# TonyLianLong/LLM-groundedDiffusion

Hardware: AMD Instinct MI355X
Metric: images/sec (50-step SD1.5 512^2, LMD+ guidance) (higher is better)
Workload: dtype fp16

## Files before the change

### llm-groundeddiffusion_amd/csrc/attn.hip

```cpp
#include <atomic>
#include "common.h"
#include "../../include/lgd_hip.h"
#include "attn_w4.h"
#include <stdlib.h>
#include <string.h>

namespace {

int g_attn32_nw = -1;
int attn32_nw() {
  if (g_attn32_nw < 0) { const char* e = getenv("LGD_ATTN32_NW"); g_attn32_nw = e ? atoi(e) : 8; }
  return g_attn32_nw;
}
int g_attn32_var = 0;
int attn32_var() { return g_attn32_var; }
int g_attn32 = -1;
int attn32_mode() {
  if (g_attn32 < 0) { const char* e = getenv("LGD_ATTN32"); g_attn32 = e ? atoi(e) : 1; }
  return g_attn32;
}

std::atomic<int> g_attn_w4{-1};
int attn_w4_mode() {
  int v = g_attn_w4.load(std::memory_order_relaxed);
// ... 791 lines not shown
    __syncthreads();
    if (t + 2 < n_tiles) load_k((t + 2) * KV_T);
    if (more) load_v((t + 1) * KV_T);
    const float mx_nxt = pipelined_tile((t + 1) & 1, t & 1, s_cur, s_nxt);
    if (more) {
      const float mx = mx_nxt;
      if (__builtin_amdgcn_ballot_w64(mx > 8.f) != 0) {
        const float m_new = (float)(half_t)fmaxf(m_ref, mx + m_ref);
        const float shift = m_new - m_ref;
        const float alpha = __builtin_amdgcn_exp2f(-shift);
#pragma unroll
        for (int dt = 0; dt < NDT; ++dt)
#pragma unroll
          for (int r = 0; r < 16; ++r) oacc[dt][r] *= alpha;
#pragma unroll
        for (int kb = 0; kb < 2; ++kb)
#pragma unroll
          for (int r = 0; r < 16; ++r) s_nxt[kb][r] -= shift;
        m_ref = m_new;
        set_ref(m_new);
      }
#pragma unroll
      for (int kb = 0; kb < 2; ++kb) s_cur[kb] = s_nxt[kb];
    }
  }

  float l;
  {
    const int dl = d & 31, dt_l = d >> 5, h_l = (dl >> 2) & 1, r_l = (dl & 3) + 4 * (dl >> 3);
    float lv = 0.f;
#pragma unroll
    for (int dt = 0; dt < NDT; ++dt)
#pragma unroll
      for (int r = 0; r < 16; ++r)
        if (dt == dt_l && r == r_l) lv = oacc[dt][r];
    l = __shfl(lv, h_l * 32 + qi, 64);
  }
  const int qrow = q0 + qi;
  if (qrow < a.Sq) {
    const float inv = 1.f / l;
    half_t* orow = a.o + (long)b * a.o_bs + (long)qrow * a.ldo + (long)h * d;
#pragma unroll
    for (int dt = 0; dt < NDT; ++dt)
#pragma unroll
      for (int g4 = 0; g4 < 4; ++g4) {
        const int dv = dt * 32 + g4 * 8 + hh * 4;
        if (dv < d) {
          half4_t o;
#pragma unroll
          for (int r = 0; r < 4; ++r) o[r] = (half_t)(oacc[dt][g4 * 4 + r] * inv);
          *reinterpret_cast<half4_t*>(orow + dv) = o;
        }
      }
    if (a.lse && hh == 0) a.lse[((long)b * a.H + h) * a.Sq + qrow] = m_ref + log2f(l);
  }
}

template <int DP, bool SAVE_P>
void launch_attn_dp(const AttnArgs& a, hipStream_t st) {
  if constexpr (SAVE_P) {
    dim3 grid((a.Sq + 63) / 64, a.H, a.B);
    hipLaunchKernelGGL((attn_fwd_kernel<DP>), grid, dim3(256), 0, st, a);
  } else {
    if constexpr (DP == 64 || DP == 96) {
      const int a32 = attn32_mode();
      const int dk = ((a.d + 2 + 15) / 16) * 16;
      const long blocks256 = (long)((a.Sq + 255) / 256) * a.H * a.B;
      if (a32 && a.d % 8 == 0 && (a32 == 2 || (dk == 96 && blocks256 >= 128))) {
        const int var = attn32_var();
        auto go = [&](auto kern, int nw) {
          dim3 g32((a.Sq + 32 * nw - 1) / (32 * nw), a.H, a.B);
          hipLaunchKernelGGL(kern, g32, dim3(64 * nw), 0, st, a);
        };
        if (attn32_nw() == 4 || (a32 != 2 && blocks256 < 256)) {
          if (dk == 48) { go(&attn_self32_kernel<48, 2, 4>, 4); return; }
          if (dk == 96) { go(&attn_self32_kernel<96, 3, 4>, 4); return; }
        } else if (var == 1) {
          if (dk == 48) { go(&attn_self32_kernel<48, 2, 8, 4, true>, 8); return; }
          if (dk == 96) { go(&attn_self32_kernel<96, 3, 8, 4, true>, 8); return; }
        } else if (var == 2) {
          if (dk == 48) { go(&attn_self32_kernel<48, 2, 8, 2, false>, 8); return; }
          if (dk == 96) { go(&attn_self32_kernel<96, 3, 8, 2, false>, 8); return; }
        } else {
          if (dk == 48) { go(&attn_self32_kernel<48, 2, 8>, 8); return; }
          if (dk == 96) { go(&attn_self32_kernel<96, 3, 8>, 8); return; }
        }
      }
    }
    const bool qt2 = (long)((a.Sq + 127) / 128) * a.H * a.B >= 1024 && DP <= 96;
    dim3 grid(qt2 ? (a.Sq + 127) / 128 : (a.Sq + 63) / 64, a.H, a.B);
    if constexpr (DP <= 96) {
      static const int nw_env = [] { const char* e = getenv("LGD_ATTN_NW"); return e ? atoi(e) : 0; }();
      const bool nw8 = nw_env ? nw_env == 8 : ((DP == 64 && a.d < 48) || DP == 96);
      if (qt2 && nw8 && (long)((a.Sq + 255) / 256) * a.H * a.B >= 512) {
        dim3 g8((a.Sq + 255) / 256, a.H, a.B);
        if (DP == 64 && a.d < 48) hipLaunchKernelGGL((attn_self_kernel<DP, true, 2, DP == 64 ? 3 : DP / 16, 8>), g8, dim3(512), 0, st, a);
        else if (a.d < DP) hipLaunchKernelGGL((attn_self_kernel<DP, true, 2, DP / 16, 8>), g8, dim3(512), 0, st, a);
        else hipLaunchKernelGGL((attn_self_kernel<DP, false, 2, DP / 16, 8>), g8, dim3(512), 0, st, a);
        return;
      }
      if (qt2) {
        if (DP == 64 && a.d < 48) hipLaunchKernelGGL((attn_self_kernel<DP, true, 2, DP == 64 ? 3 : DP / 16>), grid, dim3(256), 0, st, a);
        else if (a.d < DP) hipLaunchKernelGGL((attn_self_kernel<DP, true, 2>), grid, dim3(256), 0, st, a);
        else hipLaunchKernelGGL((attn_self_kernel<DP, false, 2>), grid, dim3(256), 0, st, a);
        return;
      }
    }
    if constexpr (DP == 160) {
      static const int wide = [] { const char* e = getenv("LGD_ATTN160"); return e ? atoi(e) : 1; }();
      if (wide && a.d == DP && a.Sq >= 256 && (long)a.H * a.B * ((a.Sq + 63) / 64) > 256) {
        dim3 g8((a.Sq + 255) / 256, a.H, a.B);
        hipLaunchKernelGGL((attn_self_kernel<DP, false, 2, DP / 16, 8>), g8, dim3(512), 0, st, a);
        return;
      }
    }
    if (DP == 64 && a.d < 48) hipLaunchKernelGGL((attn_self_kernel<DP, true, 1, DP == 64 ? 3 : DP / 16>), grid, dim3(256), 0, st, a);
    else if (a.d < DP) hipLaunchKernelGGL((attn_self_kernel<DP, true, 1>), grid, dim3(256), 0, st, a);
    else hipLaunchKernelGGL((attn_self_kernel<DP, false, 1>), grid, dim3(256), 0, st, a);
  }
}

template <bool SAVE_P>
int launch_attn(const AttnArgs& a, hipStream_t st) {
  const int d = a.d;
  if constexpr (!SAVE_P) {
    const int w4 = attn_w4_mode();
    if (w4 && d == 40) {
      AttnW4Args w;
      w.q = a.q; w.ldq = a.ldq; w.q_bs = a.q_bs; w.k = a.k; w.ldk = a.ldk; w.k_bs = a.k_bs;
      w.v = a.v; w.ldv = a.ldv; w.v_bs = a.v_bs; w.o = a.o; w.ldo = a.ldo; w.o_bs = a.o_bs; w.lse = a.lse;
      w.B = a.B; w.H = a.H; w.Sq = a.Sq; w.Sk = a.Sk; w.d = a.d; w.scale_log2 = a.scale_log2;
      const long wgs = (long)((a.Sq + 255) / 256) * a.H * a.B;
      if (lgd_attn_w4_supported(w) && (w4 == 2 || (wgs >= 256 && a.Sk >= 256))) return lgd_attn_w4_launch(w, st);
    }
  }
  if (d <= 32) launch_attn_dp<32, SAVE_P>(a, st);
  else if (d <= 64) launch_attn_dp<64, SAVE_P>(a, st);
  else if (d <= 96) launch_attn_dp<96, SAVE_P>(a, st);
  else if (d <= 128) launch_attn_dp<128, SAVE_P>(a, st);
  else if (d <= 160) launch_attn_dp<160, SAVE_P>(a, st);
  else if (d <= 192) launch_attn_dp<192, SAVE_P>(a, st);
  else return LGD_ERR_UNSUPPORTED;
  return lgd_check_launch();
}

bool bad_view(int64_t ld, int d) { return (ld % 8) != 0 || (d % 8) != 0; }

}

void lgd_gn_set_fused_hw(int hw);
void lgd_gn_set_slab(int on);
void lgd_ln_set_stream(int on);
void lgd_gn_set_apply_wgs(int n);

extern "C" int lgd_set_option(const char* name, int value) {
  if (!name) return LGD_ERR_ARG;
  if (!strcmp(name, "gn_fused") && value >= 0 && value <= 4096) { lgd_gn_set_fused_hw(value); return LGD_OK; }
  if (!strcmp(name, "gn_slab") && (value == 0 || value == 1)) { lgd_gn_set_slab(value); return LGD_OK; }
  if (!strcmp(name, "ln_stream") && (value == 0 || value == 1)) { lgd_ln_set_stream(value); return LGD_OK; }
  if (!strcmp(name, "gn_apply_wgs") && value >= 64 && value <= 8192) { lgd_gn_set_apply_wgs(value); return LGD_OK; }
  if (!strcmp(name, "attn32")) { g_attn32 = value; return LGD_OK; }
  if (!strcmp(name, "attn_w4") && value >= 0 && value <= 2) { g_attn_w4.store(value, std::memory_order_relaxed); return LGD_OK; }
  if (!strcmp(name, "attn_w4_pipe") && (value == 0 || value == 1)) { lgd_attn_w4_set_pipe(value); return LGD_OK; }
  if (!strcmp(name, "attn32_nw") && (value == 4 || value == 8)) { g_attn32_nw = value; return LGD_OK; }
  if (!strcmp(name, "attn32_var") && value >= 0 && value <= 2) { g_attn32_var = value; return LGD_OK; }
  return LGD_ERR_ARG;
}

extern "C" int lgd_attn_fwd_f16(const void* q, int64_t ldq, int64_t q_bs, const void* k,
                                int64_t ldk, int64_t k_bs, const void* v, int64_t ldv, int64_t v_bs,
                                void* o, int64_t ldo, int64_t o_bs, float* lse, int B, int H, int Sq,
                                int Sk, int d, float scale, void* stream) {
  (void)hipGetLastError();
  if (B < 1 || H < 1 || Sq < 1 || Sk < 1 || d < 8) return LGD_ERR_ARG;
  if (bad_view(ldq, d) || bad_view(ldk, d) || bad_view(ldv, d) || (ldo % 4)) return LGD_ERR_ARG;
  AttnArgs a;
  a.q = (const half_t*)q; a.ldq = ldq; a.q_bs = q_bs;
  a.k = (const half_t*)k; a.ldk = ldk; a.k_bs = k_bs;
  a.v = (const half_t*)v; a.ldv = ldv; a.v_bs = v_bs;
  a.o = (half_t*)o; a.ldo = ldo; a.o_bs = o_bs;
  a.lse = lse; a.probs = nullptr; a.tok = -1; a.cond_only = 0; a.causal = 0;
  a.B = B; a.H = H; a.Sq = Sq; a.Sk = Sk; a.d = d;
  a.scale_log2 = scale * 1.4426950408889634f;
  return launch_attn<false>(a, reinterpret_cast<hipStream_t>(stream));
}

extern "C" int lgd_cross_attn_fwd_f16(const void* q, int64_t ldq, int64_t q_bs, const void* k,
                                      int64_t ldk, int64_t k_bs, const void* v, int64_t ldv,
                                      int64_t v_bs, void* o, int64_t ldo, int64_t o_bs, float* probs,
                                      int tok, int cond_only, int B, int H, int Sq, int Sk, int d,
                                      float scale, void* stream) {
  (void)hipGetLastError();
  if (B < 1 || H < 1 || Sq < 1 || Sk < 1 || d < 8) return LGD_ERR_ARG;
  if (bad_view(ldq, d) || bad_view(ldk, d) || bad_view(ldv, d) || (ldo % 4)) return LGD_ERR_ARG;
  if (cond_only && (B % 2)) return LGD_ERR_ARG;
  if (tok >= Sk) return LGD_ERR_ARG;
  AttnArgs a;
  a.q = (const half_t*)q; a.ldq = ldq; a.q_bs = q_bs;
  a.k = (const half_t*)k; a.ldk = ldk; a.k_bs = k_bs;
  a.v = (const half_t*)v; a.ldv = ldv; a.v_bs = v_bs;
  a.o = (half_t*)o; a.ldo = ldo; a.o_bs = o_bs;
  a.lse = nullptr; a.probs = probs; a.tok = tok; a.cond_only = cond_only; a.causal = 0;
  a.B = B; a.H = H; a.Sq = Sq; a.Sk = Sk; a.d = d;
  a.scale_log2 = scale * 1.4426950408889634f;
  hipStream_t st = reinterpret_cast<hipStream_t>(stream);
  if (probs) return launch_attn<true>(a, st);
  return launch_attn<false>(a, st);
}

extern "C" int lgd_attn_causal_fwd_f16(const void* q, int64_t ldq, int64_t q_bs, const void* k, int64_t ldk,
                                       int64_t k_bs, const void* v, int64_t ldv, int64_t v_bs, void* o,
                                       int64_t ldo, int64_t o_bs, int B, int H, int S, int d, float scale,
                                       void* stream) {
  (void)hipGetLastError();
  if (B < 1 || H < 1 || S < 1 || d < 8) return LGD_ERR_ARG;
  if (bad_view(ldq, d) || bad_view(ldk, d) || bad_view(ldv, d) || (ldo % 4)) return LGD_ERR_ARG;
  AttnArgs a;
  a.q = (const half_t*)q; a.ldq = ldq; a.q_bs = q_bs;
  a.k = (const half_t*)k; a.ldk = ldk; a.k_bs = k_bs;
  a.v = (const half_t*)v; a.ldv = ldv; a.v_bs = v_bs;
  a.o = (half_t*)o; a.ldo = ldo; a.o_bs = o_bs;
  a.lse = nullptr; a.probs = nullptr; a.tok = -1; a.cond_only = 0; a.causal = 1;
  a.B = B; a.H = H; a.Sq = S; a.Sk = S; a.d = d;
  a.scale_log2 = scale * 1.4426950408889634f;
  return launch_attn<true>(a, reinterpret_cast<hipStream_t>(stream));
}
```

### llm-groundeddiffusion_amd/csrc/gemm.hip

```cpp
#include "common.h"
#include "../../include/lgd_hip.h"
#include <map>
#include <mutex>
#include <utility>
#include <stdlib.h>

namespace {

constexpr int BK = 64;
constexpr int LDS_LD = BK + 16;

struct GemmArgs {
  LgdGemmDesc d;
  int cin;
  int k_per_split;
  int group_m;
#ifdef LGD_GEMM_ABLATION
  int stagger;
#endif
};

__device__ __forceinline__ float4 ld_bias4(const float* p, int n) {
  return *reinterpret_cast<const float4*>(p + n);
}

__device__ __forceinline__ f32x4 rownorm4(const LgdGemmDesc& d, int m, int n_in, f32x4 v) {
  if (d.epi & LGD_EPI_ROWNORM) {
    const float2 st = *reinterpret_cast<const float2*>(d.rowstat + (long)m * 2);
    const float4 cs = *reinterpret_cast<const float4*>(d.colsum + n_in);
    v[0] = st.y * (v[0] - st.x * cs.x); v[1] = st.y * (v[1] - st.x * cs.y);
    v[2] = st.y * (v[2] - st.x * cs.z); v[3] = st.y * (v[3] - st.x * cs.w);
  }
  return v;
}

template <bool GEGLU>
__device__ __forceinline__ f32x4 epilogue_value4(const LgdGemmDesc& d, long r_off, int m, int n_out, f32x4 v, f32x4 g,
                                                 float4 bv, float4 bg, bool res_ready, half4_t res_pre) {
  v[0] += bv.x; v[1] += bv.y; v[2] += bv.z; v[3] += bv.w;
  if (GEGLU) {
    g[0] += bg.x; g[1] += bg.y; g[2] += bg.z; g[3] += bg.w;
#ifdef LGD_GEMM_ABLATION
    if (d.epi & (1 << 16)) {
#pragma unroll
      for (int r = 0; r < 4; ++r) v[r] = v[r] * g[r];
    } else
#endif
    {
      const f32x2_t g01 = gelu2_f((f32x2_t){g[0], g[1]}), g23 = gelu2_f((f32x2_t){g[2], g[3]});
      v[0] *= g01[0]; v[1] *= g01[1]; v[2] *= g23[0]; v[3] *= g23[1];
    }
  }
  const float alpha = d.alpha;
#pragma unroll
  for (int r = 0; r < 4; ++r) v[r] *= alpha;
  if (res_ready) {
#pragma unroll
    for (int r = 0; r < 4; ++r) v[r] += (float)res_pre[r];
  } else if (d.res) {
    if (d.epi & LGD_EPI_RES_F32) {
      const float* rp = reinterpret_cast<const float*>(d.res) + r_off + (long)m * d.ldr + n_out;
      float4 rv = *reinterpret_cast<const float4*>(rp);
      v[0] += rv.x; v[1] += rv.y; v[2] += rv.z; v[3] += rv.w;
    } else {
      const half_t* rp = reinterpret_cast<const half_t*>(d.res) + r_off + (long)m * d.ldr + n_out;
      half4_t rv = *reinterpret_cast<const half4_t*>(rp);
#pragma unroll
      for (int r = 0; r < 4; ++r) v[r] += (float)rv[r];
    }
  }
  return v;
}

template <bool GEGLU>
__device__ __forceinline__ void epilogue_store4(const LgdGemmDesc& d, long c_off, long r_off, int m,
                                                int n_out, f32x4 v, f32x4 g, float4 bv, float4 bg,
                                                bool res_ready = false,
                                                half4_t res_pre = (half4_t){0, 0, 0, 0}) {
  v = epilogue_value4<GEGLU>(d, r_off, m, n_out, v, g, bv, bg, res_ready, res_pre);
  if (d.epi & LGD_EPI_OUT_F32) {
    float* cp = reinterpret_cast<float*>(d.c) + c_off + (long)m * d.ldc + n_out;
    *reinterpret_cast<float4*>(cp) = make_float4(v[0], v[1], v[2], v[3]);
  } else {
    half_t* cp = reinterpret_cast<half_t*>(d.c) + c_off + (long)m * d.ldc + n_out;
    half4_t o;
#pragma unroll
    for (int r = 0; r < 4; ++r) o[r] = (half_t)v[r];
    *reinterpret_cast<half4_t*>(cp) = o;
  }
}

__device__ __forceinline__ float4 ld_bias_sum4(const LgdGemmDesc& d, int n) {
  float4 b = make_float4(0.f, 0.f, 0.f, 0.f);
  if (d.bias) b = ld_bias4(d.bias, n);
  if (d.bias2) {
    float4 b2 = ld_bias4(d.bias2, n);
    b.x += b2.x; b.y += b2.y; b.z += b2.z; b.w += b2.w;
  }
  return b;
}

template <int MI, int NI>
__device__ __forceinline__ void gemm_epilogue(const GemmArgs& ga, f32x4 (&acc)[NI][MI], int m0, int n0,
                                              int wm, int wn, int lane, int batch, int split,
                                              long c_off, long r_off, int* lds_flag = nullptr) {
  const LgdGemmDesc& d = ga.d;
  const int m_l = lane & 15;
  const int n_l = (lane >> 4) * 4;
  if (d.splits > 1) {
    float* ws = ga.d.ws + ((long)batch * d.splits + split) * (long)d.M * d.N;
#pragma unroll
    for (int mi = 0; mi < MI; ++mi) {
      int m = m0 + wm * 16 * MI + mi * 16 + m_l;
      if (m >= d.M) continue;
#pragma unroll
      for (int ni = 0; ni < NI; ++ni) {
        int n = n0 + wn * 16 * NI + ni * 16 + n_l;
        if (n >= d.N) continue;
        f32x4 v = acc[ni][mi];
        *reinterpret_cast<float4*>(ws + (long)m * d.N + n) = make_float4(v[0], v[1], v[2], v[3]);
      }
    }
    if (!d.cnt || !lds_flag) return;
    asm volatile("s_waitcnt vmcnt(0)" ::: "memory");
    __syncthreads();
    int32_t* cnt = d.cnt + (long)batch * gridDim.x + blockIdx.x;
    if (threadIdx.x == 0) {
      __builtin_amdgcn_fence(__ATOMIC_RELEASE, "agent");
      asm volatile("s_waitcnt vmcnt(0)" ::: "memory");
      *lds_flag = __hip_atomic_fetch_add(cnt, 1, __ATOMIC_RELAXED, __HIP_MEMORY_SCOPE_AGENT);
    }
    __syncthreads();
    if (*lds_flag != d.splits - 1) return;
    if (threadIdx.x == 0) {
      __builtin_amdgcn_fence(__ATOMIC_ACQUIRE, "agent");
      __hip_atomic_store(cnt, 0, __ATOMIC_RELAXED, __HIP_MEMORY_SCOPE_AGENT);
    }
    __syncthreads();
    const float* w0 = ga.d.ws + (long)batch * d.splits * (long)d.M * d.N;
#pragma unroll
    for (int mi = 0; mi < MI; ++mi) {
      const int m = m0 + wm * 16 * MI + mi * 16 + m_l;
#pragma unroll
      for (int ni = 0; ni < NI; ++ni) {
        const int n = n0 + wn * 16 * NI + ni * 16 + n_l;
        f32x4 v = {0.f, 0.f, 0.f, 0.f};
        if (m < d.M && n < d.N) {
          for (int s2 = 0; s2 < d.splits; ++s2) {
            const float4 t = *reinterpret_cast<const float4*>(w0 + (long)s2 * d.M * d.N + (long)m * d.N + n);
            v[0] += t.x; v[1] += t.y; v[2] += t.z; v[3] += t.w;
          }
        }
        acc[ni][mi] = v;
      }
    }
  }
  const bool geglu = d.epi & LGD_EPI_GEGLU;
  if (geglu) {
// ... 1258 lines not shown
  const int frow = lane & 15, fg = lane >> 4, fsw = (frow >> 1) & 7;
  const unsigned lds0 = (unsigned)(uintptr_t)smem;
  unsigned a_ad0 = lds0 + (grp * 16 * MH + frow) * 128 + ((0 + fg) ^ fsw) * 16;
  unsigned a_ad1 = lds0 + (grp * 16 * MH + frow) * 128 + ((4 + fg) ^ fsw) * 16;
  unsigned b_ad0 = lds0 + OFF_B0 + (wn * 16 + frow) * 128 + ((0 + fg) ^ fsw) * 16;
  unsigned b_ad1 = lds0 + OFF_B0 + (wn * 16 + frow) * 128 + ((4 + fg) ^ fsw) * 16;
  using seqA = std::make_integer_sequence<int, MH>;
  using seqB0 = std::make_integer_sequence<int, NI0>;
  using seqB1 = std::make_integer_sequence<int, NI1>;

  f32x4 acc[NI][MI];
  half8_t af[2][MH], bf0[2][NI0], bf1[2][NI1];
  if constexpr (ABL & 2) {
#pragma unroll
    for (int kk = 0; kk < 2; ++kk) {
#pragma unroll
      for (int i = 0; i < MH; ++i) af[kk][i] = (half8_t){1, 1, 1, 1, 1, 1, 1, 1};
#pragma unroll
      for (int i = 0; i < NI0; ++i) bf0[kk][i] = (half8_t){1, 1, 1, 1, 1, 1, 1, 1};
#pragma unroll
      for (int i = 0; i < NI1; ++i) bf1[kk][i] = (half8_t){1, 1, 1, 1, 1, 1, 1, 1};
    }
  }

#define LGD_PH_MMA(BF, NB, NOFF, MOFF)                                                                              \
  {                                                                                                                 \
    asm volatile("s_waitcnt lgkmcnt(0)" ::: "memory");                                                              \
    __builtin_amdgcn_sched_barrier(0);                                                                              \
    if constexpr (!(ABL & 32)) __builtin_amdgcn_s_setprio(1);                                                       \
    _Pragma("unroll") for (int kk = 0; kk < 2; ++kk)                                                                \
      _Pragma("unroll") for (int ni = 0; ni < NB; ++ni)                                                             \
        _Pragma("unroll") for (int mi = 0; mi < MH; ++mi)                                                           \
          if constexpr (ABL & 4) asm volatile("" : "+v"(acc[NOFF + ni][MOFF + mi]) : "v"(BF[kk][ni]), "v"(af[kk][mi]));                \
          else acc[NOFF + ni][MOFF + mi] = __builtin_amdgcn_mfma_f32_16x16x32_f16(BF[kk][ni], af[kk][mi], acc[NOFF + ni][MOFF + mi], 0, 0, 0); \
    if constexpr (!(ABL & 32)) __builtin_amdgcn_s_setprio(0);                                                       \
    __builtin_amdgcn_sched_barrier(0);                                                                              \
  }
#define LGD_PH_BAR()                        \
  {                                         \
    __builtin_amdgcn_sched_barrier(0);      \
    __builtin_amdgcn_s_barrier();           \
    __builtin_amdgcn_sched_barrier(0);      \
  }

  if (nk > 0) {
    {
      unsigned sa, sw; int tap;
      k_pos(0, sa, sw, tap);
      dma_b(0, 0, true, sw, false);
      dma_a(0, 0, true, sa, tap, false);
      dma_b(1, 0, true, sw, false);
      dma_a(1, 0, true, sa, tap, false);
      k_pos(1, sa, sw, tap);
      dma_b(0, STAGE_B, nk > 1, sw, false);
      dma_a(0, STAGE_B, nk > 1, sa, tap, false);
    }
#pragma unroll
    for (int ni = 0; ni < NI; ++ni)
#pragma unroll
      for (int mi = 0; mi < MI; ++mi) acc[ni][mi] = (f32x4){0.f, 0.f, 0.f, 0.f};
    asm volatile("s_waitcnt vmcnt(%0)" ::"n"(T_DMA) : "memory");
    LGD_PH_BAR();
    if (grp == 1 && !(ABL & 64)) LGD_PH_BAR();
    unsigned so_cur = 0, so_nxt = STAGE_B;
    int sdelta = STAGE_B;
    for (int kt = 0; kt < nk; ++kt) {
      unsigned sa1, sw1, sa2, sw2; int tap1, tap2;
      k_pos(kt + 1, sa1, sw1, tap1);
      k_pos(kt + 2, sa2, sw2, tap2);
      const bool live1 = kt + 1 < nk, live2 = kt + 2 < nk;
      if constexpr (!(ABL & 2)) lds_read_frags<0, 64 * 128>(bf0[0], b_ad0, seqB0{});
      if constexpr (!(ABL & 2)) lds_read_frags<0, 64 * 128>(bf0[1], b_ad1, seqB0{});
      if constexpr (!(ABL & 2)) lds_read_frags<0, 16 * 128>(af[0], a_ad0, seqA{});
      if constexpr (!(ABL & 2)) lds_read_frags<0, 16 * 128>(af[1], a_ad1, seqA{});
      dma_b(1, so_nxt, live1, sw1);
      asm volatile("s_waitcnt vmcnt(%0)" ::"n"(T_DMA) : "memory");
      LGD_PH_BAR();
      LGD_PH_MMA(bf0, NI0, 0, 0);
      LGD_PH_BAR();
      if constexpr (!(ABL & 2)) lds_read_frags<BQ0_B, 64 * 128>(bf1[0], b_ad0, seqB1{});
      if constexpr (!(ABL & 2)) lds_read_frags<BQ0_B, 64 * 128>(bf1[1], b_ad1, seqB1{});
      dma_a(1, so_nxt, live1, sa1, tap1);
      asm volatile("s_waitcnt vmcnt(%0)" ::"n"(T_DMA) : "memory");
      LGD_PH_BAR();
      LGD_PH_MMA(bf1, NI1, NI0, 0);
      LGD_PH_BAR();
      if constexpr (!(ABL & 2)) lds_read_frags<OFF_A1, 16 * 128>(af[0], a_ad0, seqA{});
      if constexpr (!(ABL & 2)) lds_read_frags<OFF_A1, 16 * 128>(af[1], a_ad1, seqA{});
      dma_b(0, so_cur, live2, sw2);
      LGD_PH_BAR();
      LGD_PH_MMA(bf1, NI1, NI0, MH);
      LGD_PH_BAR();
      dma_a(0, so_cur, live2, sa2, tap2);
      asm volatile("s_waitcnt vmcnt(%0)" ::"n"(T_DMA) : "memory");
      LGD_PH_BAR();
      LGD_PH_MMA(bf0, NI0, 0, MH);
      LGD_PH_BAR();
      a_ad0 += sdelta; a_ad1 += sdelta; b_ad0 += sdelta; b_ad1 += sdelta;
      sdelta = -sdelta;
      const unsigned t = so_cur; so_cur = so_nxt; so_nxt = t;
    }
    if (grp == 0 && !(ABL & 64)) LGD_PH_BAR();
    asm volatile("s_waitcnt vmcnt(0) lgkmcnt(0)" ::: "memory");
    LGD_PH_BAR();
  }
  else {
#pragma unroll
    for (int ni = 0; ni < NI; ++ni)
#pragma unroll
      for (int mi = 0; mi < MI; ++mi) acc[ni][mi] = (f32x4){0.f, 0.f, 0.f, 0.f};
  }
#undef LGD_PH_MMA
#undef LGD_PH_BAR

  if constexpr (ABL & 16) {
#pragma unroll
    for (int ni = 0; ni < NI; ++ni)
#pragma unroll
      for (int mi = 0; mi < MI; ++mi) asm volatile("" ::"v"(acc[ni][mi]));
    return;
  }
  if (d.splits > 1) {
    const int m_l = lane & 15, n_l = (lane >> 4) * 4;
    float* ws = d.ws + ((long)batch * d.splits + split) * (long)d.M * d.N;
#pragma unroll
    for (int mi = 0; mi < MI; ++mi) {
      const int m = m0 + grp * 16 * MI + mi * 16 + m_l;
      if (m >= d.M) continue;
#pragma unroll
      for (int ni = 0; ni < NI; ++ni) {
        const int n = n0 + wn * 16 * NI + ni * 16 + n_l;
        if (n >= d.N) continue;
        const f32x4 v = acc[ni][mi];
        *reinterpret_cast<float4*>(ws + (long)m * d.N + n) = make_float4(v[0], v[1], v[2], v[3]);
      }
    }
    return;
  }
#define LGD_EPI_LDS(G, RS, RNORM) \
  gemm_epilogue_lds<MI, NI, WM, WN, (MI * NI > 32 ? STAGE_B : 2 * STAGE_B), G, true, RS, RNORM>(ga, acc, m0, n0, grp, wn, lane, tid, c_off, r_off, lds)
  const bool rn_ = d.epi & LGD_EPI_ROWNORM;
  if (d.epi & LGD_EPI_GEGLU) {
    if constexpr (NI % 2 == 0) {
      if (rn_) LGD_EPI_LDS(true, false, true); else LGD_EPI_LDS(true, false, false);
    }
  } else if (d.res) {
    if (rn_) LGD_EPI_LDS(false, true, true); else LGD_EPI_LDS(false, true, false);
  } else {
    if (rn_) LGD_EPI_LDS(false, false, true); else LGD_EPI_LDS(false, false, false);
  }
#undef LGD_EPI_LDS
}

__global__ __launch_bounds__(256) void splitk_reduce_kernel(const GemmArgs ga) {
  const LgdGemmDesc& d = ga.d;
  const bool geglu = d.epi & LGD_EPI_GEGLU;
  const int n_out_cols = geglu ? d.N / 2 : d.N;
  const long groups_per_row = n_out_cols / 4;
  const long total = (long)d.M * groups_per_row;
  const int batch = blockIdx.z;
  const int b_o = batch / d.nb_i, b_i = batch - b_o * d.nb_i;
  const long c_off = b_o * d.c_bs_o + b_i * d.c_bs_i;
  const long r_off = b_o * d.r_bs_o + b_i * d.r_bs_i;
  const float* ws = d.ws + (long)batch * d.splits * (long)d.M * d.N;
  for (long idx = blockIdx.x * 256L + threadIdx.x; idx < total; idx += (long)gridDim.x * 256L) {
    int m = (int)(idx / groups_per_row);
    int gcol = (int)(idx - (long)m * groups_per_row) * 4;
    int n_in = geglu ? (gcol / 16) * 32 + (gcol % 16) : gcol;
    f32x4 v = {0.f, 0.f, 0.f, 0.f}, g = {0.f, 0.f, 0.f, 0.f};
    for (int s = 0; s < d.splits; ++s) {
      const float* p = ws + (long)s * d.M * d.N + (long)m * d.N + n_in;
      float4 t = *reinterpret_cast<const float4*>(p);
      v[0] += t.x; v[1] += t.y; v[2] += t.z; v[3] += t.w;
      if (geglu) {
        float4 u = *reinterpret_cast<const float4*>(p + 16);
        g[0] += u.x; g[1] += u.y; g[2] += u.z; g[3] += u.w;
      }
    }
    const float4 bv = ld_bias_sum4(d, n_in);
    v = rownorm4(d, m, n_in, v);
    if (geglu) {
      float4 bg = make_float4(0.f, 0.f, 0.f, 0.f);
      if (d.bias) bg = ld_bias4(d.bias, n_in + 16);
      epilogue_store4<true>(d, c_off, r_off, m, gcol, v, rownorm4(d, m, n_in + 16, g), bv, bg);
    } else {
      epilogue_store4<false>(d, c_off, r_off, m, gcol, v, g, bv, bv);
    }
  }
}

enum GemmLoop : int {
  LOOP_REG,
  LOOP_DMA,
  LOOP_DMA8,
  LOOP_PIPE,
  LOOP_PHASE,
};
enum : unsigned {
  TILE_GEGLU = 1,
  TILE_PLAIN = 2,
  TILE_ONE_SPLIT = 4,
  TILE_LDS_EPI = 8,
  TILE_CONV_SAME = 16,
  TILE_CNT = 32,
};
struct GemmTile {
  int code;
  GemmLoop loop;
  int bm, bn;
  unsigned flags;
};
constexpr unsigned TILE_STD = TILE_GEGLU | TILE_CNT;
constexpr GemmTile GEMM_TILES[] = {
    {1, LOOP_REG, 128, 128, TILE_STD},   {2, LOOP_REG, 128, 64, TILE_STD},     {3, LOOP_REG, 64, 128, TILE_STD},
    {4, LOOP_REG, 64, 64, TILE_STD},     {5, LOOP_REG, 32, 128, TILE_STD},     {6, LOOP_REG, 128, 160, TILE_CNT},
    {7, LOOP_REG, 64, 160, TILE_CNT},
    {17, LOOP_DMA, 128, 128, TILE_STD},  {18, LOOP_DMA, 128, 64, TILE_STD},    {19, LOOP_DMA, 64, 128, TILE_STD},
    {20, LOOP_DMA, 64, 64, TILE_STD},    {21, LOOP_DMA, 32, 128, TILE_STD},    {22, LOOP_DMA, 128, 160, TILE_CNT},
    {23, LOOP_DMA, 64, 160, TILE_CNT},
    {25, LOOP_DMA8, 256, 320, TILE_CNT}, {26, LOOP_DMA8, 256, 128, TILE_STD},
    {33, LOOP_PIPE, 256, 160, TILE_CNT}, {34, LOOP_PIPE, 256, 128, TILE_STD}, {35, LOOP_PIPE, 256, 64, TILE_STD},
    {37, LOOP_PIPE, 128, 160, TILE_CNT}, {38, LOOP_PIPE, 128, 128, TILE_STD}, {39, LOOP_PIPE, 128, 64, TILE_STD},
    {40, LOOP_PIPE, 64, 160, TILE_CNT},  {41, LOOP_PIPE, 64, 128, TILE_STD},  {42, LOOP_PIPE, 64, 64, TILE_STD},
    {44, LOOP_PIPE, 256, 256, TILE_GEGLU | TILE_PLAIN | TILE_ONE_SPLIT | TILE_LDS_EPI},
    {45, LOOP_PIPE, 128, 128, TILE_STD | TILE_PLAIN},
    {46, LOOP_PHASE, 256, 256, TILE_GEGLU | TILE_LDS_EPI | TILE_CONV_SAME},
    {47, LOOP_PHASE, 256, 320, TILE_LDS_EPI | TILE_CONV_SAME},
};

const GemmTile* gemm_check(const LgdGemmDesc& desc, GemmArgs& ga) {
  ga.d = desc;
  LgdGemmDesc& d = ga.d;
  if (d.M <= 0 || d.N <= 0 || d.K <= 0) return nullptr;
  if (d.taps != 1 && d.taps != 9) return nullptr;
  ga.cin = d.c0 + d.c1;
  if (d.K != d.taps * ga.cin) return nullptr;
  if ((d.c0 % 8) || (d.c1 % 8) || (d.N % 4) || (d.ldw % 8) || (d.lda0 % 8) || (d.lda1 % 8) ||
      (d.ldc % 4))
    return nullptr;
  if (d.c1 > 0 && !d.a1) return nullptr;
  if (d.res && (d.ldr % 4)) return nullptr;
  if (d.nb_o < 1) d.nb_o = 1;
  if (d.nb_i < 1) d.nb_i = 1;
  if (d.splits < 1) d.splits = 1;
  const bool geglu = d.epi & LGD_EPI_GEGLU;
  if (geglu && (d.N % 32)) return nullptr;
  if (d.splits > 1 && !d.ws) return nullptr;
  if ((d.epi & LGD_EPI_ROWNORM) && (!d.rowstat || !d.colsum || d.taps != 1 || d.nb_o * d.nb_i != 1 || d.c1 > 0))
    return nullptr;
  int ktiles = (d.K + BK - 1) / BK;
  int tps = (ktiles + d.splits - 1) / d.splits;
  ga.k_per_split = tps * BK;
  d.splits = (ktiles + tps - 1) / tps;

  int code = d.tile;
  if (code == 0) {
    long batches = (long)d.nb_o * d.nb_i * d.splits;
    auto wgs = [&](int bm, int bn) {
      return batches * ((d.M + bm - 1) / bm) * ((d.N + bn - 1) / bn);
    };
    if (d.M <= 32) code = 21;
    else if (!geglu && d.N % 160 == 0 && wgs(128, 160) >= 384) code = 22;
    else if (!geglu && d.N % 160 == 0 && wgs(64, 160) >= 256) code = 23;
    else if (wgs(128, 128) >= 384 && d.N % 128 == 0) code = 17;
    else if (wgs(64, 128) >= 256 && d.N % 128 == 0) code = 19;
    else code = 20;
  }
  const GemmTile* t = nullptr;
  for (const GemmTile& e : GEMM_TILES)
    if (e.code == code) t = &e;
  if (!t) return nullptr;
  const unsigned f = t->flags;
  if (geglu && !(f & TILE_GEGLU)) return nullptr;
  if (t->loop == LOOP_DMA8 && (d.K % BK)) return nullptr;
  if ((t->loop == LOOP_PIPE || t->loop == LOOP_PHASE) && ((d.K % BK) || (ga.cin % BK) || (d.c0 % BK))) return nullptr;
  if ((f & TILE_PLAIN) && (d.taps != 1 || d.c1 > 0)) return nullptr;
  if (t->loop == LOOP_PHASE) {
    if (d.c1 > 0 || d.nb_o * d.nb_i != 1) return nullptr;
    if (((long)d.M + 2L * d.win + 2) * d.lda0 * 2 + 2L * d.K >= (1L << 31) || (long)d.N * d.ldw * 2 >= (1L << 31))
      return nullptr;
  }
  if ((f & TILE_CONV_SAME) && d.taps == 9 && (d.stride != 1 || d.ups != 0 || d.hin != d.hout || d.win != d.wout))
    return nullptr;
  if ((f & TILE_ONE_SPLIT) && d.splits != 1) return nullptr;
  if ((f & TILE_LDS_EPI) && d.splits == 1) {
    const long c_off_max = (long)(d.nb_o - 1) * d.c_bs_o + (long)(d.nb_i - 1) * d.c_bs_i;
    if ((d.epi & LGD_EPI_OUT_F32) || (d.N & 7) || (d.ldc & 7) || (c_off_max & 7) || (d.c_bs_o & 7) || (d.c_bs_i & 7) ||
        (reinterpret_cast<uintptr_t>(d.c) & 15) || (d.res && (d.epi & (LGD_EPI_RES_F32 | LGD_EPI_GEGLU))))
      return nullptr;
  }
  if (d.splits > 1 && d.cnt && !(f & TILE_CNT)) return nullptr;
  return t;
}

using GemmKernel = void (*)(GemmArgs);

int lds_kernel(GemmKernel kern, int smem, int threads, long* resident = nullptr) {
  static std::mutex mu;
  static std::map<std::pair<GemmKernel, int>, long> ready;
  int dev = 0;
  if (hipGetDevice(&dev) != hipSuccess) return LGD_ERR_LAUNCH;
  std::lock_guard<std::mutex> lock(mu);
  auto it = ready.find({kern, dev});
  if (it == ready.end()) {
    if (hipFuncSetAttribute(reinterpret_cast<const void*>(kern), hipFuncAttributeMaxDynamicSharedMemorySize, smem) !=
        hipSuccess)
      return LGD_ERR_LAUNCH;
    it = ready.emplace(std::make_pair(kern, dev), -1L).first;
  }
  if (resident) {
    if (it->second < 0) {
      int per_cu = 0, cus = 0;
      if (hipDeviceGetAttribute(&cus, hipDeviceAttributeMultiprocessorCount, dev) != hipSuccess ||
          hipOccupancyMaxActiveBlocksPerMultiprocessor(&per_cu, reinterpret_cast<const void*>(kern), threads, smem) !=
              hipSuccess)
        return LGD_ERR_LAUNCH;
      it->second = (long)(cus / 8) * 8 * (per_cu > 0 ? per_cu : 1);
    }
    *resident = it->second;
  }
  return LGD_OK;
}

template <int MI, int NI, int WM = 2>
int launch_gemm(const GemmArgs& ga, hipStream_t st, bool dma) {
  constexpr int BM = WM * 16 * MI, BN = 32 * NI;
  const LgdGemmDesc& d = ga.d;
  long tiles = (long)((d.M + BM - 1) / BM) * ((d.N + BN - 1) / BN);
  dim3 grid((unsigned)tiles, 1, (unsigned)(d.nb_o * d.nb_i * d.splits));
  if constexpr (WM == 2) {
    if (dma) hipLaunchKernelGGL((gemm_dma_kernel<MI, NI, 2>), grid, dim3(256), 0, st, ga);
    else hipLaunchKernelGGL((gemm_kernel<MI, NI>), grid, dim3(256), 0, st, ga);
  } else {
    hipLaunchKernelGGL((gemm_dma_kernel<MI, NI, WM>), grid, dim3(128 * WM), 0, st, ga);
  }
  return lgd_check_launch();
}

template <int MI, int NI, int WM, int WN, int NS, bool CM>
int launch_gemm_pipe_cm(const GemmArgs& ga, hipStream_t st) {
  constexpr int BM = WM * 16 * MI, BN = WN * 16 * NI;
  constexpr int SMEM = NS * (BM + BN) * BK * 2;
  constexpr int THREADS = 64 * WM * WN;
  constexpr bool HAS_PERSIST = !CM && !(MI == 4 && NI == 5) && NS != 2;
  const LgdGemmDesc& d = ga.d;
  long tiles = (long)((d.M + BM - 1) / BM) * ((d.N + BN - 1) / BN);
  GemmKernel kern = &gemm_pipe_kernel<MI, NI, WM, WN, NS, CM>;
  long resident = 0;
  if constexpr (HAS_PERSIST) {
    static const bool persist_on = [] { const char* e = getenv("LGD_GEMM_PERSIST"); return !(e && e[0] == '0'); }();
    if (persist_on)
      if (int rc = lds_kernel(&gemm_pipe_kernel<MI, NI, WM, WN, NS, false, true>, SMEM, THREADS, &resident)) return rc;
  }
  const bool persist = resident > 0 && d.nb_o * d.nb_i * d.splits == 1 && tiles > resident && d.K <= 10 * BK && d.taps == 1;
  dim3 grid((unsigned)(persist ? resident : tiles), 1, (unsigned)(d.nb_o * d.nb_i * d.splits));
  if constexpr (HAS_PERSIST)
    if (persist) kern = &gemm_pipe_kernel<MI, NI, WM, WN, NS, false, true>;
#ifdef LGD_GEMM_ABLATION
  static const int abl = [] { const char* e = getenv("LGD_GEMM_ABL"); return e ? atoi(e) : 0; }();
  if (abl) {
    switch (abl) {
      case 1: kern = &gemm_pipe_kernel<MI, NI, WM, WN, NS, CM, false, 1>; break;
      case 2: kern = &gemm_pipe_kernel<MI, NI, WM, WN, NS, CM, false, 2>; break;
      case 3: kern = &gemm_pipe_kernel<MI, NI, WM, WN, NS, CM, false, 3>; break;
      case 4: kern = &gemm_pipe_kernel<MI, NI, WM, WN, NS, CM, false, 4>; break;
      case 6: kern = &gemm_pipe_kernel<MI, NI, WM, WN, NS, CM, false, 6>; break;
      case 8: kern = &gemm_pipe_kernel<MI, NI, WM, WN, NS, CM, false, 8>; break;
      case 11: kern = &gemm_pipe_kernel<MI, NI, WM, WN, NS, CM, false, 11>; break;
      case 16: kern = &gemm_pipe_kernel<MI, NI, WM, WN, NS, CM, false, 16>; break;
      case 17: kern = &gemm_pipe_kernel<MI, NI, WM, WN, NS, CM, false, 17>; break;
      case 20: kern = &gemm_pipe_kernel<MI, NI, WM, WN, NS, CM, false, 20>; break;
      default: return lgd_check_launch();
    }
  }
#endif
  if (int rc = lds_kernel(kern, SMEM, THREADS)) return rc;
  hipLaunchKernelGGL(kern, grid, dim3(THREADS), SMEM, st, ga);
  return lgd_check_launch();
}

template <int MI, int NI, int WM, int WN, int NS>
int launch_gemm_pipe(const GemmArgs& ga, hipStream_t st) {
  const LgdGemmDesc& d = ga.d;
  static const int no_cm = [] { const char* e = getenv("LGD_GEMM_NO_CM"); return (e && e[0] == '1') ? 1 : 0; }();
  if constexpr (NS != 2) {
    if (d.taps == 9 && d.stride == 1 && d.ups == 0 && d.c1 == 0 && !no_cm)
      return launch_gemm_pipe_cm<MI, NI, WM, WN, NS, true>(ga, st);
  }
  return launch_gemm_pipe_cm<MI, NI, WM, WN, NS, false>(ga, st);
}

template <int MI, int NI>
int launch_gemm_phase(const GemmArgs& ga, hipStream_t st) {
  constexpr int BM = 32 * MI, BN = 64 * NI;
  constexpr int SMEM = 2 * (BM + BN) * BK * 2;
  const LgdGemmDesc& d = ga.d;
  const bool conv = d.taps == 9;
  long tiles = (long)((d.M + BM - 1) / BM) * ((d.N + BN - 1) / BN);
  dim3 grid((unsigned)tiles, 1, (unsigned)(d.nb_o * d.nb_i * d.splits));
  GemmKernel kern = conv ? &gemm_phase_kernel<MI, NI, true> : &gemm_phase_kernel<MI, NI, false>;
#ifdef LGD_GEMM_ABLATION
  static const int abl = [] { const char* e = getenv("LGD_GEMM_ABL"); return e ? atoi(e) : 0; }();
  if (abl) {
#define LGD_PH_ABL(A) case A: kern = conv ? &gemm_phase_kernel<MI, NI, true, A> : &gemm_phase_kernel<MI, NI, false, A>; break;
    switch (abl) {
      LGD_PH_ABL(1) LGD_PH_ABL(2) LGD_PH_ABL(3) LGD_PH_ABL(4) LGD_PH_ABL(6) LGD_PH_ABL(16) LGD_PH_ABL(17) LGD_PH_ABL(20) LGD_PH_ABL(32) LGD_PH_ABL(64) LGD_PH_ABL(96)
      default: return lgd_check_launch();
    }
#undef LGD_PH_ABL
  }
#endif
  if (int rc = lds_kernel(kern, SMEM, 512)) return rc;
  hipLaunchKernelGGL(kern, grid, dim3(512), SMEM, st, ga);
  return lgd_check_launch();
}

int launch_tile(const GemmTile& t, const GemmArgs& ga, hipStream_t st) {
  const bool dma = t.loop == LOOP_DMA && ga.d.K % BK == 0;
  switch (t.code) {
    case 33: return launch_gemm_pipe<4, 5, 4, 2, 3>(ga, st);
    case 34: return launch_gemm_pipe<4, 4, 4, 2, 3>(ga, st);
    case 35: return launch_gemm_pipe<4, 2, 4, 2, 4>(ga, st);
    case 37: return launch_gemm_pipe<2, 5, 4, 2, 4>(ga, st);
    case 38: return launch_gemm_pipe<2, 4, 4, 2, 4>(ga, st);
    case 39: return launch_gemm_pipe<2, 2, 4, 2, 5>(ga, st);
    case 40: return launch_gemm_pipe<1, 5, 4, 2, 5>(ga, st);
    case 41: return launch_gemm_pipe<1, 4, 4, 2, 5>(ga, st);
    case 42: return launch_gemm_pipe<1, 2, 4, 2, 6>(ga, st);
    case 44: return launch_gemm_pipe<4, 8, 4, 2, 2>(ga, st);
    case 45: return launch_gemm_pipe<2, 4, 4, 2, 2>(ga, st);
    case 46: return launch_gemm_phase<8, 4>(ga, st);
    case 47: return launch_gemm_phase<8, 5>(ga, st);
    case 1: case 17: return launch_gemm<4, 4>(ga, st, dma);
    case 2: case 18: return launch_gemm<4, 2>(ga, st, dma);
    case 3: case 19: return launch_gemm<2, 4>(ga, st, dma);
    case 4: case 20: return launch_gemm<2, 2>(ga, st, dma);
    case 5: case 21: return launch_gemm<1, 4>(ga, st, dma);
    case 6: case 22: return launch_gemm<4, 5>(ga, st, dma);
    case 7: case 23: return launch_gemm<2, 5>(ga, st, dma);
    case 25: return launch_gemm<4, 10, 4>(ga, st, true);
    case 26: return launch_gemm<4, 4, 4>(ga, st, true);
  }
  return LGD_ERR_ARG;
}

}

extern "C" int lgd_abi_version(void) { return LGD_ABI_VERSION; }

extern "C" int lgd_gemm_check(const LgdGemmDesc* desc) {
  GemmArgs ga;
  return desc && gemm_check(*desc, ga) ? LGD_OK : LGD_ERR_ARG;
}

extern "C" int lgd_gemm_f16(const LgdGemmDesc* desc, void* stream) {
  (void)hipGetLastError();
  GemmArgs ga;
  const GemmTile* t = desc ? gemm_check(*desc, ga) : nullptr;
  if (!t) return LGD_ERR_ARG;
  const LgdGemmDesc& d = ga.d;
  hipStream_t st = reinterpret_cast<hipStream_t>(stream);
#ifdef LGD_GEMM_ABLATION
  { const char* e = getenv("LGD_GEMM_STAGGER"); ga.stagger = e ? atoi(e) : 0; }
#endif
  {
    static const int forced = [] { const char* e = getenv("LGD_GEMM_GROUP_M"); return e ? atoi(e) : 0; }();
    ga.group_m = 1;
    const long w_bytes = (long)d.N * d.K * 2;
    if (d.taps == 1 && d.nb_o * d.nb_i == 1 && w_bytes > (5L << 19)) {
      long g = (3L << 20) / (256L * d.K * 2);
      ga.group_m = forced > 0 ? forced : (int)(g < 1 ? 1 : g > 8 ? 8 : g);
    }
  }
  int rc = launch_tile(*t, ga, st);
  if (rc || d.splits == 1 || d.cnt) return rc;
  int n_out = (d.epi & LGD_EPI_GEGLU) ? d.N / 2 : d.N;
  long total = (long)d.M * (n_out / 4);
  int blocks = (int)((total + 255) / 256);
  if (blocks > 2048) blocks = 2048;
  dim3 grid(blocks, 1, d.nb_o * d.nb_i);
  hipLaunchKernelGGL(splitk_reduce_kernel, grid, dim3(256), 0, st, ga);
  return lgd_check_launch();
}
```

Baseline: 1.932.

## Add persistent GEMM kernel keeping whole A panel resident in LDS for small-K

Adds a persistent GEMM kernel for large-M, small-K (K up to 320), wide-N non-conv GEMMs. Each workgroup loads its full 128-row A panel for all K into LDS once, then sweeps N tiles while double-buffering only B. The epilogue is staged through LDS and written with buffer stores. The aim is to stop re-fetching A for every N tile and to cut per-tile launch and prologue cost. The trade-off is a large LDS footprint (one workgroup per CU), a narrow dispatch condition, and no support for batch or residual offsets beyond zero.

```diff
diff --git a/llm-groundeddiffusion_amd/csrc/attn.hip b/llm-groundeddiffusion_amd/csrc/attn.hip
--- a/llm-groundeddiffusion_amd/csrc/attn.hip
+++ b/llm-groundeddiffusion_amd/csrc/attn.hip
@@ -967,6 +967,7 @@
 void lgd_gn_set_slab(int on);
 void lgd_ln_set_stream(int on);
 void lgd_gn_set_apply_wgs(int n);
+void lgd_gemm_set_astat(int on);
 
 extern "C" int lgd_set_option(const char* name, int value) {
   if (!name) return LGD_ERR_ARG;
@@ -974,6 +975,7 @@
   if (!strcmp(name, "gn_slab") && (value == 0 || value == 1)) { lgd_gn_set_slab(value); return LGD_OK; }
   if (!strcmp(name, "ln_stream") && (value == 0 || value == 1)) { lgd_ln_set_stream(value); return LGD_OK; }
   if (!strcmp(name, "gn_apply_wgs") && value >= 64 && value <= 8192) { lgd_gn_set_apply_wgs(value); return LGD_OK; }
+  if (!strcmp(name, "gemm_astat") && (value == 0 || value == 1)) { lgd_gemm_set_astat(value); return LGD_OK; }
   if (!strcmp(name, "attn32")) { g_attn32 = value; return LGD_OK; }
   if (!strcmp(name, "attn_w4") && value >= 0 && value <= 2) { g_attn_w4.store(value, std::memory_order_relaxed); return LGD_OK; }
   if (!strcmp(name, "attn_w4_pipe") && (value == 0 || value == 1)) { lgd_attn_w4_set_pipe(value); return LGD_OK; }
diff --git a/llm-groundeddiffusion_amd/csrc/gemm.hip b/llm-groundeddiffusion_amd/csrc/gemm.hip
--- a/llm-groundeddiffusion_amd/csrc/gemm.hip
+++ b/llm-groundeddiffusion_amd/csrc/gemm.hip
@@ -1,9 +1,13 @@
 #include "common.h"
 #include "../../include/lgd_hip.h"
+#include <atomic>
 #include <map>
 #include <mutex>
 #include <utility>
 #include <stdlib.h>
+
+std::atomic<int> g_gemm_astat{1};
+void lgd_gemm_set_astat(int on) { g_gemm_astat.store(on, std::memory_order_relaxed); }
 
 namespace {
 
@@ -1568,6 +1572,273 @@
 #undef LGD_EPI_LDS
 }
 
+constexpr int ASTAT_BM = 128, ASTAT_BN = 256, ASTAT_MAX_KT = 5;
+constexpr int ASTAT_A_KT = ASTAT_BM * BK * 2;
+constexpr int ASTAT_STAGE = ASTAT_BN * BK * 2;
+constexpr int ASTAT_OFF_B = ASTAT_MAX_KT * ASTAT_A_KT;
+constexpr int ASTAT_SMEM = ASTAT_OFF_B + 2 * ASTAT_STAGE;
+static_assert(ASTAT_SMEM <= 160 * 1024, "LDS");
+
+typedef unsigned u32x4_t __attribute__((ext_vector_type(4)));
+template <bool GEGLU>
+constexpr int astat_epi_stores() {
+  constexpr int BN_OUT = GEGLU ? ASTAT_BN / 2 : ASTAT_BN, CROW = BN_OUT * 2 + 16;
+  constexpr int R = (ASTAT_BM * CROW <= ASTAT_STAGE) ? 1 : ((ASTAT_BM / 2) * CROW <= ASTAT_STAGE) ? 2 : 4;
+  return R * (ASTAT_BM / R) * (BN_OUT / 8) / 512;
+}
+template <bool GEGLU, bool RES16, bool RN>
+__device__ __forceinline__ void astat_epilogue(const LgdGemmDesc& d, f32x4 (&acc)[4][4], int m0, int n0, int wm, int wn,
+                                               int lane, int tid, unsigned char* lds) {
+  static_assert(!(GEGLU && RES16), "GEGLU outputs take no residual here");
+  constexpr int MI = 4, NI = 4, NT = 512;
+  constexpr int BN_OUT = GEGLU ? ASTAT_BN / 2 : ASTAT_BN;
+  constexpr int NI_OUT = GEGLU ? NI / 2 : NI;
+  constexpr int CROW = BN_OUT * 2 + 16;
+  constexpr int R = (ASTAT_BM * CROW <= ASTAT_STAGE) ? 1 : ((ASTAT_BM / 2) * CROW <= ASTAT_STAGE) ? 2 : 4;
+  constexpr int MI_R = MI / R, WROWS = 16 * MI_R, RROWS = 2 * WROWS, CPR = BN_OUT / 8;
+  constexpr int PER = RROWS * CPR / NT;
+  static_assert(RROWS * CPR % NT == 0 && R * PER == astat_epi_stores<GEGLU>(), "store count");
+  const int m_l = lane & 15, n_l = (lane >> 4) * 4;
+  const int n0_out = GEGLU ? n0 / 2 : n0;
+  const int n_total_out = GEGLU ? d.N / 2 : d.N;
+  const f32x2_t alpha2 = {d.alpha, d.alpha};
+  float4 bv[NI_OUT], bg[NI_OUT], cv[NI_OUT], cg[NI_OUT];
+  int mrow[MI];
+  float2 st[MI];
+  half4_t rpre[NI_OUT][MI];
+#pragma unroll
+  for (int no = 0; no < NI_OUT; ++no) {
+    const int n_out = n0_out + wn * 16 * NI_OUT + no * 16 + n_l;
+    const int n_in = GEGLU ? n0 + wn * 16 * NI + no * 32 + n_l : n_out;
+    bv[no] = make_float4(0.f, 0.f, 0.f, 0.f);
+    bg[no] = bv[no];
+    cv[no] = bv[no];
+    cg[no] = bv[no];
+    if (n_out < n_total_out) {
+      bv[no] = ld_bias_sum4(d, n_in);
+      if (GEGLU && d.bias) bg[no] = ld_bias4(d.bias, n_in + 16);
+      if constexpr (RN) {
+        cv[no] = *reinterpret_cast<const float4*>(d.colsum + n_in);
+        if (GEGLU) cg[no] = *reinterpret_cast<const float4*>(d.colsum + n_in + 16);
+      }
+    }
+  }
+#pragma unroll
+  for (int mi = 0; mi < MI; ++mi) {
+    int m = m0 + wm * 16 * MI + mi * 16 + m_l;
+    if (m >= d.M) m = d.M - 1;
+    mrow[mi] = m;
+    st[mi] = make_float2(0.f, 1.f);
+    if constexpr (RN) st[mi] = *reinterpret_cast<const float2*>(d.rowstat + (long)m * 2);
+  }
+  if constexpr (RES16) {
+    const half_t* rb = reinterpret_cast<const half_t*>(d.res);
+#pragma unroll
+    for (int mi = 0; mi < MI; ++mi)
+#pragma unroll
+      for (int no = 0; no < NI_OUT; ++no) {
+        const int n_out = n0_out + wn * 16 * NI_OUT + no * 16 + n_l;
+        rpre[no][mi] = *reinterpret_cast<const half4_t*>(rb + (long)mrow[mi] * d.ldr + (n_out < n_total_out ? n_out : 0));
+      }
+  }
+  auto normed = [&](const f32x4& v, const float2 s2, const float4 c, const float4 b, f32x2_t& lo, f32x2_t& hi) {
+    lo = (f32x2_t){v[0], v[1]};
+    hi = (f32x2_t){v[2], v[3]};
+    if constexpr (RN) {
+      const f32x2_t mean = {s2.x, s2.x}, rstd = {s2.y, s2.y};
+      lo = rstd * (lo - mean * (f32x2_t){c.x, c.y});
+      hi = rstd * (hi - mean * (f32x2_t){c.z, c.w});
+    }
+    lo += (f32x2_t){b.x, b.y};
+    hi += (f32x2_t){b.z, b.w};
+  };
+  constexpr unsigned OOB = 0x80000000u;
+  const __amdgpu_buffer_rsrc_t rc = __builtin_amdgcn_make_buffer_rsrc(d.c, 0, 0x80000000u, 0x00020000);
+  const unsigned ldc2 = (unsigned)d.ldc * 2u;
+  unsigned char* lw = lds + (wm * WROWS + m_l) * CROW + (wn * 16 * NI_OUT + n_l) * 2;
+#pragma unroll
+  for (int r = 0; r < R; ++r) {
+#pragma unroll
+    for (int no = 0; no < NI_OUT; ++no) {
+#pragma unroll
+      for (int mj = 0; mj < MI_R; ++mj) {
+        const int mi = r * MI_R + mj;
+        f32x2_t lo, hi;
+        if constexpr (GEGLU) {
+          f32x2_t glo, ghi;
+          normed(acc[2 * no][mi], st[mi], cv[no], bv[no], lo, hi);
+          normed(acc[2 * no + 1][mi], st[mi], cg[no], bg[no], glo, ghi);
+          lo *= gelu2_f(glo); hi *= gelu2_f(ghi);
+        } else {
+          normed(acc[no][mi], st[mi], cv[no], bv[no], lo, hi);
+        }
+        lo *= alpha2;
+        hi *= alpha2;
+        if constexpr (RES16) {
+          const half4_t rr = rpre[no][mi];
+          lo += (f32x2_t){(float)rr[0], (float)rr[1]};
+          hi += (f32x2_t){(float)rr[2], (float)rr[3]};
+        }
+        const half4_t o = {(half_t)lo[0], (half_t)lo[1], (half_t)hi[0], (half_t)hi[1]};
+        *reinterpret_cast<half4_t*>(lw + mj * 16 * CROW + no * 32) = o;
+      }
+    }
+    asm volatile("s_waitcnt lgkmcnt(0)" ::: "memory");
+    __builtin_amdgcn_s_barrier();
+#pragma unroll
+    for (int i = 0; i < PER; ++i) {
+      const int idx = tid + i * NT;
+      const int row = idx / CPR, ch = idx - row * CPR;
+      const int wr = row / WROWS;
+      const int m = m0 + wr * 16 * MI + r * WROWS + (row - wr * WROWS), n = n0_out + ch * 8;
+      const uint4 val = *reinterpret_cast<const uint4*>(lds + row * CROW + ch * 16);
+      const unsigned vo = m < d.M && n < n_total_out ? (unsigned)m * ldc2 + (unsigned)n * 2u : OOB;
+      __builtin_amdgcn_raw_buffer_store_b128((u32x4_t){val.x, val.y, val.z, val.w}, rc, vo, 0, 0);
+    }
+    if (r + 1 < R) {
+      asm volatile("s_waitcnt lgkmcnt(0)" ::: "memory");
+      __builtin_amdgcn_s_barrier();
+    }
+  }
+}
+
+__global__ __launch_bounds__(512, 1) void gemm_astat_kernel(const GemmArgs ga) {
+  constexpr int MI = 4, NI = 4, WM = 2, WN = 4;
+  static_assert(WM * 16 * MI == ASTAT_BM && WN * 16 * NI == ASTAT_BN, "tile");
+  constexpr int NB = ASTAT_BN / 64;
+  constexpr unsigned OOB = 0x80000000u;
+  constexpr unsigned NREC = 0x80000000u;
+
+  extern __shared__ __attribute__((aligned(1024))) half_t smem[];
+  unsigned char* lds = reinterpret_cast<unsigned char*>(smem);
+
+  const LgdGemmDesc& d = ga.d;
+  const int tid = threadIdx.x;
+  const int lane = tid & 63;
+  const int wid = __builtin_amdgcn_readfirstlane(tid >> 6);
+  const int grp = wid >> 2, wn = wid & 3;
+
+  const int n_tiles = (d.N + ASTAT_BN - 1) / ASTAT_BN;
+  const long work = (long)((d.M + ASTAT_BM - 1) / ASTAT_BM) * n_tiles;
+  const int w_beg = __builtin_amdgcn_readfirstlane((int)(work * blockIdx.x / gridDim.x));
+  const int w_end = __builtin_amdgcn_readfirstlane((int)(work * (blockIdx.x + 1) / gridDim.x));
+  const int nk = __builtin_amdgcn_readfirstlane(d.K / BK);
+  const int steps = (w_end - w_beg) * nk;
+  constexpr long c_off = 0, r_off = 0;
+
+  const int lrow = lane >> 3;
+  const int kseg = (lane & 7) ^ ((((wid & 1) << 2) + (lrow >> 1)) & 7);
+  const unsigned lda2 = (unsigned)d.lda0 * 2u, ldw2 = (unsigned)d.ldw * 2u;
+  const int row8 = wid * 8 + lrow;
+  const half_t* a_base = reinterpret_cast<const half_t*>(d.a0);
+  const half_t* w_base = reinterpret_cast<const half_t*>(d.w);
+  const unsigned voffB = (unsigned)row8 * ldw2 + kseg * 16;
+  auto dma_a = [&](int m0) {
+    const __amdgpu_buffer_rsrc_t rs = __builtin_amdgcn_make_buffer_rsrc(const_cast<half_t*>(a_base), 0, NREC, 0x00020000);
+#pragma unroll
+    for (int j = 0; j < 2; ++j) {
+      const unsigned vo = m0 + 64 * j + row8 < d.M ? (unsigned)(m0 + row8) * lda2 + kseg * 16 : OOB;
+      for (int kt = 0; kt < nk; ++kt)
+        __builtin_amdgcn_raw_ptr_buffer_load_lds(rs, (lds_ptr_t)(lds + kt * ASTAT_A_KT + (j * 8 + wid) * 1024), 16, vo,
+                                                 (unsigned)(kt * BK * 2) + (unsigned)(64 * j) * lda2, 0, 0);
+    }
+  };
+  auto dma_b = [&](int n0, int kt, unsigned so) {
+    const __amdgpu_buffer_rsrc_t rs = __builtin_amdgcn_make_buffer_rsrc(const_cast<half_t*>(w_base), 0, NREC, 0x00020000);
+#pragma unroll
+    for (int i = 0; i < NB; ++i) {
+      const unsigned vo = n0 + 64 * i + row8 < d.N ? voffB : OOB;
+      __builtin_amdgcn_raw_ptr_buffer_load_lds(rs, (lds_ptr_t)(lds + ASTAT_OFF_B + so + (i * 8 + wid) * 1024), 16, vo,
+                                               (unsigned)(n0 + 64 * i) * ldw2 + (unsigned)(kt * BK * 2), 0, 0);
+    }
+  };
+
+  const int frow = lane & 15, fg = lane >> 4, fsw = (frow >> 1) & 7;
+  const unsigned lds0 = (unsigned)(uintptr_t)smem;
+  const unsigned a_ad0 = lds0 + (grp * 64 + frow) * 128 + ((0 + fg) ^ fsw) * 16;
+  const unsigned a_ad1 = lds0 + (grp * 64 + frow) * 128 + ((4 + fg) ^ fsw) * 16;
+  const unsigned b_ad0 = lds0 + ASTAT_OFF_B + (wn * 64 + frow) * 128 + ((0 + fg) ^ fsw) * 16;
+  const unsigned b_ad1 = lds0 + ASTAT_OFF_B + (wn * 64 + frow) * 128 + ((4 + fg) ^ fsw) * 16;
+  using seqA = std::make_integer_sequence<int, MI>;
+  using seqB = std::make_integer_sequence<int, NI>;
+
+#define LGD_AS_BAR()                        \
+  {                                         \
+    __builtin_amdgcn_sched_barrier(0);      \
+    __builtin_amdgcn_s_barrier();           \
+    __builtin_amdgcn_sched_barrier(0);      \
+  }
+
+  f32x4 acc[NI][MI];
+#pragma unroll
+  for (int ni = 0; ni < NI; ++ni)
+#pragma unroll
+    for (int mi = 0; mi < MI; ++mi) acc[ni][mi] = (f32x4){0.f, 0.f, 0.f, 0.f};
+  if (steps > 0) {
+    int panel = w_beg / n_tiles, tile = w_beg - panel * n_tiles, kt = 0;
+    unsigned so = 0;
+    bool epi_stores = false;
+    dma_a(panel * ASTAT_BM);
+    dma_b(tile * ASTAT_BN, 0, 0);
+    for (int g = 0; g < steps; ++g) {
+      if (!epi_stores) asm volatile("s_waitcnt vmcnt(0)" ::: "memory");
+      else asm volatile("s_waitcnt vmcnt(%0)" ::"n"(astat_epi_stores<false>()) : "memory");
+      epi_stores = false;
+      LGD_AS_BAR();
+      if (kt == 0 && g > 0 && tile == 0) {
+        dma_a(panel * ASTAT_BM);
+        asm volatile("s_waitcnt vmcnt(0)" ::: "memory");
+        LGD_AS_BAR();
+      }
+      if (g + 1 < steps) {
+        if (kt + 1 < nk) dma_b(tile * ASTAT_BN, kt + 1, so ^ ASTAT_STAGE);
+        else dma_b(tile + 1 < n_tiles ? (tile + 1) * ASTAT_BN : 0, 0, so ^ ASTAT_STAGE);
+      }
+      const unsigned ka = kt * ASTAT_A_KT;
+      half8_t af[2][MI], bf[2][NI];
+      lds_read_frags<0, 16 * 128>(bf[0], b_ad0 + so, seqB{});
+      lds_read_frags<0, 16 * 128>(af[0], a_ad0 + ka, seqA{});
+      wait_frags<-1>(af[0], bf[0]);
+      lds_read_frags<0, 16 * 128>(bf[1], b_ad1 + so, seqB{});
+      lds_read_frags<0, 16 * 128>(af[1], a_ad1 + ka, seqA{});
+      __builtin_amdgcn_sched_barrier(0);
+#pragma unroll
+      for (int ni = 0; ni < NI; ++ni)
+#pragma unroll
+        for (int mi = 0; mi < MI; ++mi)
+          acc[ni][mi] = __builtin_amdgcn_mfma_f32_16x16x32_f16(bf[0][ni], af[0][mi], acc[ni][mi], 0, 0, 0);
+      wait_frags<-1>(af[1], bf[1]);
+#pragma unroll
+      for (int ni = 0; ni < NI; ++ni)
+#pragma unroll
+        for (int mi = 0; mi < MI; ++mi)
+          acc[ni][mi] = __builtin_amdgcn_mfma_f32_16x16x32_f16(bf[1][ni], af[1][mi], acc[ni][mi], 0, 0, 0);
+      if (++kt == nk) {
+        LGD_AS_BAR();
+        unsigned char* stage = lds + ASTAT_OFF_B + so;
+        const int m0 = panel * ASTAT_BM, n0 = tile * ASTAT_BN;
+#define LGD_EPI_AS(G, RS, RNORM) astat_epilogue<G, RS, RNORM>(d, acc, m0, n0, grp, wn, lane, tid, stage)
+        const bool rn_ = d.epi & LGD_EPI_ROWNORM;
+        if (d.res) {
+          if (rn_) LGD_EPI_AS(false, true, true); else LGD_EPI_AS(false, true, false);
+        } else {
+          if (rn_) LGD_EPI_AS(false, false, true); else LGD_EPI_AS(false, false, false);
+        }
+#undef LGD_EPI_AS
+        epi_stores = true;
+#pragma unroll
+        for (int ni = 0; ni < NI; ++ni)
+#pragma unroll
+          for (int mi = 0; mi < MI; ++mi) acc[ni][mi] = (f32x4){0.f, 0.f, 0.f, 0.f};
+        kt = 0;
+        if (++tile == n_tiles) { tile = 0; ++panel; }
+      }
+      so ^= ASTAT_STAGE;
+    }
+  }
+#undef LGD_AS_BAR
+}
+
 __global__ __launch_bounds__(256) void splitk_reduce_kernel(const GemmArgs ga) {
   const LgdGemmDesc& d = ga.d;
   const bool geglu = d.epi & LGD_EPI_GEGLU;
@@ -1806,12 +2077,26 @@
   return launch_gemm_pipe_cm<MI, NI, WM, WN, NS, false>(ga, st);
 }
 
+int launch_gemm_astat(const GemmArgs& ga, hipStream_t st) {
+  const LgdGemmDesc& d = ga.d;
+  GemmKernel kern = &gemm_astat_kernel;
+  long resident = 0;
+  if (int rc = lds_kernel(kern, ASTAT_SMEM, 512, &resident)) return rc;
+  const long work = (long)((d.M + ASTAT_BM - 1) / ASTAT_BM) * ((d.N + ASTAT_BN - 1) / ASTAT_BN);
+  dim3 grid((unsigned)(work < resident ? work : resident));
+  hipLaunchKernelGGL(kern, grid, dim3(512), ASTAT_SMEM, st, ga);
+  return lgd_check_launch();
+}
+
 template <int MI, int NI>
 int launch_gemm_phase(const GemmArgs& ga, hipStream_t st) {
   constexpr int BM = 32 * MI, BN = 64 * NI;
   constexpr int SMEM = 2 * (BM + BN) * BK * 2;
   const LgdGemmDesc& d = ga.d;
   const bool conv = d.taps == 9;
+  if (NI == 5 && !conv && d.splits == 1 && d.K <= ASTAT_MAX_KT * BK && d.N >= 960 && d.M >= 32768 &&
+      (long)d.M * d.ldc * 2 < (1L << 31) && g_gemm_astat.load(std::memory_order_relaxed))
+    return launch_gemm_astat(ga, st);
   long tiles = (long)((d.M + BM - 1) / BM) * ((d.N + BN - 1) / BN);
   dim3 grid((unsigned)tiles, 1, (unsigned)(d.nb_o * d.nb_i * d.splits));
   GemmKernel kern = conv ? &gemm_phase_kernel<MI, NI, true> : &gemm_phase_kernel<MI, NI, false>;
```

Measured after the change: 1.923 (median of 6 runs). Within noise of the previous version (-0.5%).
